# openhome/ohPipeline

Hardware: AMD Instinct MI355X
Metric: PCM Msamples/s, 256-stream 44.1->48k S24 resample+ramp+fmt (higher is better)
Workload: dtype int32

## Files before the change

include/ohgpu.h:

```cpp
#ifndef OHGPU_H
#define OHGPU_H

#include <stddef.h>
#include <stdint.h>

#ifdef __cplusplus
extern "C" {
#endif

#define OHGPU_ABI_VERSION 1

#define OHGPU_OK                0
#define OHGPU_ERR_INVALID      (-1)
#define OHGPU_ERR_DEVICE       (-2)
#define OHGPU_ERR_NO_DEVICE    (-3)
#define OHGPU_ERR_NOMEM        (-4)
#define OHGPU_ERR_BOUNDS       (-5)
#define OHGPU_ERR_UNSUPPORTED  (-6)

#define OHGPU_ENDIAN_LITTLE 1
#define OHGPU_ENDIAN_BIG    2

#define OHGPU_RAMP_MAX 16384u
#define OHGPU_UNITY_ATTENUATION 256u
// ... 800 lines not shown

int ohgpu_dsd_file_batch_check(const ohgpu_dsd_file_stream_desc* descs, size_t n, uint64_t src_arena_bytes, uint64_t dst_arena_bytes);
int ohgpu_dsd_file_batch_create(ohgpu_ctx* ctx, const ohgpu_dsd_file_stream_desc* descs, size_t n, uint64_t src_arena_bytes, uint64_t dst_arena_bytes,
                                ohgpu_batch** batch);
int ohgpu_dsd_file_batch_run(ohgpu_ctx* ctx, const ohgpu_batch* batch, const void* src_base, void* dst_base, void* stream);
int ohgpu_dsd_file_batch_results(ohgpu_ctx* ctx, const ohgpu_batch* batch, ohgpu_dsd_file_stream_result* results, size_t n);
int ohgpu_dsd_file_batch_phase_ms(ohgpu_ctx* ctx, const ohgpu_batch* batch, float ms[2]);
int ohgpu_dsd_file_process_host(ohgpu_ctx* ctx, const ohgpu_dsd_file_stream_desc* descs, size_t n, const void* src_host, uint64_t src_bytes,
                                void* dst_host, uint64_t dst_bytes, ohgpu_dsd_file_stream_result* results);
int ohgpu_dsd_file_head(const void* bytes, uint64_t n, uint32_t sample_block_words, uint32_t pad_bytes_per_chunk, ohgpu_dsd_file_stream_result* result);
int ohgpu_dsd_file_seek(uint32_t kind, uint64_t sample, uint64_t* chunk_first, uint64_t* sample_rounded);

int ohgpu_src_design(uint32_t rate_in, uint32_t rate_out, uint32_t taps_per_phase, double beta, double f_pass_hz,
                     int32_t* coef_q28, size_t coef_capacity, uint32_t* L, uint32_t* M);
int ohgpu_src_create(ohgpu_ctx* ctx, uint32_t L, uint32_t M, uint32_t taps_per_phase, const int32_t* coef_q28, ohgpu_src** src);
int ohgpu_src_destroy(ohgpu_ctx* ctx, ohgpu_src* src);
uint64_t ohgpu_src_out_frames(uint32_t L, uint32_t M, uint64_t in_frames);
int ohgpu_src_mfma_tables(uint32_t L, uint32_t M, uint32_t taps_per_phase, const int32_t* coef_q28, uint32_t max_blocks_per_row,
                          uint8_t* coef_digits, size_t coef_digits_capacity, void* steps, size_t steps_capacity,
                          size_t* coef_digits_bytes, size_t* steps_bytes, uint32_t* block_outputs);
int ohgpu_src_mfma_halfband_tables(const int32_t* coef_q28 , uint8_t* image , int64_t* bias, uint32_t* block_outputs);
int ohgpu_src_batch_create(ohgpu_ctx* ctx, const ohgpu_src* src, const ohgpu_src_msg_desc* descs, size_t n,
                           uint64_t src_arena_bytes, uint64_t dst_arena_bytes, ohgpu_batch** batch);
int ohgpu_src_batch_run(ohgpu_ctx* ctx, const ohgpu_batch* batch, const void* src_base, void* dst_base, void* stream);
int ohgpu_src_batch_run_timed(ohgpu_ctx* ctx, const ohgpu_batch* batch, const void* src_base, void* dst_base, void* stream,
                              void* start_event, void* stop_event);

int ohgpu_src_batch_block(const ohgpu_batch* batch, uint32_t* block_outputs, uint32_t* block_inputs);
int ohgpu_src_batch_advance(ohgpu_ctx* ctx, ohgpu_batch* batch, uint64_t blocks);
int ohgpu_src_batch_set_ramps(ohgpu_ctx* ctx, ohgpu_batch* batch, const uint16_t* ramp_start, const uint16_t* ramp_end, size_t n);

int ohgpu_src_process_host(ohgpu_ctx* ctx, const ohgpu_src* src, const ohgpu_src_msg_desc* descs, size_t n,
                           const void* src_host, uint64_t src_bytes, void* dst_host, uint64_t dst_bytes);

#define OHGPU_SRC_PULL_NOMINAL     (1u << 31)
#define OHGPU_SRC_PULL_MAX_STEP    (16ull << 32)

typedef struct ohgpu_src_pull_msg_desc {
    uint64_t src_offset;
    uint64_t src_frame0;
    uint64_t src_frames;
    uint64_t pos_frame;
    uint64_t step;
    uint64_t dst_offset;
    uint32_t pos_frac;
    uint32_t n_frames;
    uint16_t ramp_start;
    uint16_t ramp_end;
    uint16_t attenuation;
    uint8_t  channels;
    uint8_t  src_bits;
    uint8_t  src_endian;
    uint8_t  dst_bits;
    uint8_t  dst_endian;
    uint8_t  flags;
    uint8_t  reserved[4];
    uint64_t src_plane_stride;
} ohgpu_src_pull_msg_desc;

int ohgpu_src_pull_design(uint32_t rate_in, uint32_t rate_out, uint32_t taps_per_phase, uint32_t phases_log2, double beta,
                          double f_pass_hz, double max_pull, int32_t* coef_q28, size_t coef_capacity);
int ohgpu_src_pull_step(uint32_t rate_in, uint32_t rate_out, uint32_t multiplier, uint64_t* step);
int ohgpu_src_pull_window(uint64_t pos_frame, uint32_t pos_frac, uint64_t step, uint32_t n_frames, uint32_t taps_per_phase,
                          uint64_t* first, uint64_t* frames);
int ohgpu_src_pull_create(ohgpu_ctx* ctx, uint32_t taps_per_phase, uint32_t phases_log2, const int32_t* coef_q28, ohgpu_src** src);
int ohgpu_src_pull_destroy(ohgpu_ctx* ctx, ohgpu_src* src);
// ... 40 lines not shown
```

ohpipeline_amd/capi.py:

```python
import ctypes as C
import os

import numpy as np

_PKG = os.path.dirname(os.path.abspath(__file__))
LIB_PATH = os.path.join(_PKG, "lib", "libohgpu.so")

OK = 0
ERR_INVALID, ERR_DEVICE, ERR_NO_DEVICE, ERR_NOMEM, ERR_BOUNDS, ERR_UNSUPPORTED = -1, -2, -3, -4, -5, -6
ENDIAN_LITTLE, ENDIAN_BIG = 1, 2
RAMP_MAX = 16384
UNITY_ATTENUATION = 256
FLAG_RAMP, FLAG_SILENCE, FLAG_ZERO_LSB32, FLAG_SRC_PLANAR32 = 1, 2, 4, 8

MSG_DESC = np.dtype([
    ("src_offset", "<u8"), ("dst_offset", "<u8"), ("n_frames", "<u4"),
    ("ramp_start", "<u2"), ("ramp_end", "<u2"), ("attenuation", "<u2"),
    ("channels", "u1"), ("src_bits", "u1"), ("src_endian", "u1"),
    ("dst_bits", "u1"), ("dst_endian", "u1"), ("flags", "u1")], align=False)
SRC_MSG_DESC = np.dtype([
    ("src_offset", "<u8"), ("src_frame0", "<u8"), ("src_frames", "<u8"), ("out_frame0", "<u8"),
    ("dst_offset", "<u8"), ("n_frames", "<u4"),
    ("ramp_start", "<u2"), ("ramp_end", "<u2"), ("attenuation", "<u2"),
    ("channels", "u1"), ("src_bits", "u1"), ("src_endian", "u1"),
# ... 295 lines not shown
                                              C.c_size_t, C.POINTER(C.c_size_t)]),
    "ohgpu_flywheel_batch_create": (C.c_int, [_vp, _vp, C.c_size_t, C.c_uint64, C.c_uint64, _vpp]),
    "ohgpu_flywheel_batch_run": (C.c_int, [_vp, _vp, _vp, _vp, _vp]),
    "ohgpu_flywheel_process_host": (C.c_int, [_vp, _vp, C.c_size_t, _vp, C.c_uint64, _vp, C.c_uint64]),
    "ohgpu_ohm_frame_layout": (C.c_int, [_vp, C.c_uint32, C.POINTER(C.c_uint32), C.POINTER(C.c_uint32)]),
    "ohgpu_ohm_batch_create": (C.c_int, [_vp, _vp, C.c_size_t, _vp, C.c_size_t, _vp, C.c_size_t, C.c_uint64, C.c_uint64, _vpp]),
    "ohgpu_ohm_batch_run": (C.c_int, [_vp, _vp, _vp, _vp, _vp]),
    "ohgpu_ohm_process_host": (C.c_int, [_vp, _vp, C.c_size_t, _vp, C.c_size_t, _vp, C.c_size_t, _vp, C.c_uint64, _vp, C.c_uint64]),
    "ohgpu_src_design": (C.c_int, [C.c_uint32, C.c_uint32, C.c_uint32, C.c_double, C.c_double, _vp, C.c_size_t,
                                   C.POINTER(C.c_uint32), C.POINTER(C.c_uint32)]),
    "ohgpu_src_create": (C.c_int, [_vp, C.c_uint32, C.c_uint32, C.c_uint32, _vp, _vpp]),
    "ohgpu_src_destroy": (C.c_int, [_vp, _vp]),
    "ohgpu_src_out_frames": (C.c_uint64, [C.c_uint32, C.c_uint32, C.c_uint64]),
    "ohgpu_src_mfma_tables": (C.c_int, [C.c_uint32, C.c_uint32, C.c_uint32, _vp, C.c_uint32, _vp, C.c_size_t, _vp, C.c_size_t,
                                        C.POINTER(C.c_size_t), C.POINTER(C.c_size_t), C.POINTER(C.c_uint32)]),
    "ohgpu_src_mfma_halfband_tables": (C.c_int, [_vp, _vp, C.POINTER(C.c_int64), C.POINTER(C.c_uint32)]),
    "ohgpu_src_batch_create": (C.c_int, [_vp, _vp, _vp, C.c_size_t, C.c_uint64, C.c_uint64, _vpp]),
    "ohgpu_src_batch_run": (C.c_int, [_vp, _vp, _vp, _vp, _vp]),
    "ohgpu_src_batch_run_timed": (C.c_int, [_vp, _vp, _vp, _vp, _vp, _vp, _vp]),
    "ohgpu_src_batch_plan": (C.c_int, [_vp, _u64p, _u64p]),
    "ohgpu_src_batch_units": (C.c_int, [_vp, _u64p, _u64p]),
    "ohgpu_set_plan_threads": (C.c_int, [C.c_int]),
    "ohgpu_src_batch_block": (C.c_int, [_vp, C.POINTER(C.c_uint32), C.POINTER(C.c_uint32)]),
    "ohgpu_src_batch_advance": (C.c_int, [_vp, _vp, C.c_uint64]),
    "ohgpu_src_batch_set_ramps": (C.c_int, [_vp, _vp, _vp, _vp, C.c_size_t]),
    "ohgpu_src_plan_digest": (C.c_int, [C.c_uint32, C.c_uint32, C.c_uint32, _vp, C.c_size_t, C.c_uint64, C.c_uint64, C.c_int,
                                        _vp, C.c_int, _u64p, _u64p, _u64p, C.POINTER(C.c_int)]),
    "ohgpu_src_batch_kernel_name": (C.c_int, [_vp, _vp, C.c_char_p, C.c_size_t]),
    "ohgpu_src_batch_occupancy": (C.c_int, [_vp, _vp, C.POINTER(C.c_int), C.POINTER(C.c_int), C.POINTER(C.c_uint32)]),
    "ohgpu_measure_shader_clock": (C.c_int, [_vp, _vp, C.POINTER(C.c_double)]),
    "ohgpu_device_allocations": (C.c_int, [_vp, C.POINTER(C.c_uint64)]),
    "ohgpu_src_process_host": (C.c_int, [_vp, _vp, _vp, C.c_size_t, _vp, C.c_uint64, _vp, C.c_uint64]),
    "ohgpu_host_transfer_stats": (C.c_int, [_vp, C.POINTER(C.c_uint64), C.POINTER(C.c_uint64), C.POINTER(C.c_uint64), C.POINTER(C.c_uint64)]),
    "ohgpu_set_kernel_variant": (C.c_int, [_vp, C.c_int]),
    "ohgpu_src_pull_design": (C.c_int, [C.c_uint32, C.c_uint32, C.c_uint32, C.c_uint32, C.c_double, C.c_double, C.c_double, _vp, C.c_size_t]),
    "ohgpu_src_pull_step": (C.c_int, [C.c_uint32, C.c_uint32, C.c_uint32, _u64p]),
    "ohgpu_src_pull_window": (C.c_int, [C.c_uint64, C.c_uint32, C.c_uint64, C.c_uint32, C.c_uint32, _u64p, _u64p]),
    "ohgpu_src_pull_create": (C.c_int, [_vp, C.c_uint32, C.c_uint32, _vp, _vpp]),
    "ohgpu_src_pull_destroy": (C.c_int, [_vp, _vp]),
    "ohgpu_src_pull_batch_create": (C.c_int, [_vp, _vp, _vp, C.c_size_t, C.c_uint64, C.c_uint64, _vpp]),
    "ohgpu_src_pull_batch_run": (C.c_int, [_vp, _vp, _vp, _vp, _vp]),
    "ohgpu_src_pull_process_host": (C.c_int, [_vp, _vp, _vp, C.c_size_t, _vp, C.c_uint64, _vp, C.c_uint64]),
}
CENC_SYMBOLS = {
    "ohgpu_cenc_batch_check": (C.c_int, [_vp, C.c_size_t, C.c_size_t, C.c_size_t, C.c_uint64, C.c_uint64]),
    "ohgpu_cenc_batch_create": (C.c_int, [_vp, _vp, C.c_size_t, C.c_size_t, C.c_size_t, C.c_uint64, C.c_uint64, _vpp]),
    "ohgpu_cenc_batch_run": (C.c_int, [_vp, _vp, _vp, _vp, _vp]),
    "ohgpu_cenc_batch_results": (C.c_int, [_vp, _vp, _vp, C.c_size_t]),
    "ohgpu_cenc_batch_runs": (C.c_int, [_vp, _vp, _vp, C.c_size_t]),
    "ohgpu_cenc_batch_packets": (C.c_int, [_vp, _vp, _vp, C.c_size_t]),
    "ohgpu_cenc_batch_samples": (C.c_int, [_vp, _vp, _vp, C.c_size_t]),
    "ohgpu_cenc_batch_phase_ms": (C.c_int, [_vp, _vp, C.POINTER(C.c_float)]),
    "ohgpu_cenc_batch_paths": (C.c_int, [_vp, C.POINTER(C.c_uint32), C.POINTER(C.c_uint32), C.POINTER(C.c_uint32)]),
    "ohgpu_cenc_head": (C.c_int, [_vp, C.c_size_t, _vp]),
    "ohgpu_cenc_process_host": (C.c_int, [_vp, _vp, C.c_size_t, C.c_size_t, C.c_size_t, _vp, C.c_uint64, _vp, C.c_uint64, _vp, _vp, _vp, _vp]),
    "ohgpu_cenc_flac_process_host": (C.c_int, [_vp, _vp, _vp, C.c_size_t, C.c_size_t, C.c_size_t, _vp, C.c_uint64, C.c_uint64, _vp, C.c_uint64, _vp, _vp, _vp, _vp, _vp, _vp,
                                               C.c_size_t, C.POINTER(C.c_size_t)]),
    "ohgpu_cenc_alac_process_host": (C.c_int, [_vp, _vp, _vp, C.c_size_t, C.c_size_t, C.c_size_t, _vp, C.c_uint64, C.c_uint64, _vp, C.c_uint64, _vp, _vp, _vp, _vp, _vp, _vp]),
}
RAOP_RX_SYMBOLS = {
    "ohgpu_raop_rx_batch_check": (C.c_int, [_vp, C.c_size_t, _vp, C.c_size_t, C.c_uint64]),
    "ohgpu_raop_rx_batch_create": (C.c_int, [_vp, _vp, C.c_size_t, _vp, C.c_size_t, C.c_uint64, _vpp]),
    "ohgpu_raop_rx_batch_run": (C.c_int, [_vp, _vp, _vp, _vp]),
    "ohgpu_raop_rx_batch_results": (C.c_int, [_vp, _vp, _vp, C.c_size_t, _vp, C.c_size_t]),
    "ohgpu_raop_rx_batch_packets": (C.c_int, [_vp, _vp, _vp, C.c_size_t]),
    "ohgpu_raop_rx_batch_phase_ms": (C.c_int, [_vp, _vp, C.POINTER(C.c_float)]),
# ... 1276 lines not shown
    def src_destroy(self, src):
        check(lib().ohgpu_src_destroy(self._h, src))

    def src_batch(self, src, descs, src_arena_bytes, dst_arena_bytes):
        d = np.ascontiguousarray(descs)
        assert d.dtype == SRC_MSG_DESC
        b = C.c_void_p()
        check(lib().ohgpu_src_batch_create(self._h, src, d.ctypes.data_as(C.c_void_p), d.size, src_arena_bytes,
                                           dst_arena_bytes, C.byref(b)))
        return b

    def src_batch_block(self, batch):
        lo, mi = C.c_uint32(0), C.c_uint32(0)
        check(lib().ohgpu_src_batch_block(batch, C.byref(lo), C.byref(mi)))
        return int(lo.value), int(mi.value)

    def src_batch_advance(self, batch, blocks):
        check(lib().ohgpu_src_batch_advance(self._h, batch, blocks))

    def src_batch_set_ramps(self, batch, ramp_start, ramp_end):
        a = np.ascontiguousarray(ramp_start, dtype=np.uint16)
        e = np.ascontiguousarray(ramp_end, dtype=np.uint16)
        assert a.size == e.size
        check(lib().ohgpu_src_batch_set_ramps(self._h, batch, a.ctypes.data_as(C.c_void_p), e.ctypes.data_as(C.c_void_p), a.size))

    def src_process_host(self, src, descs, src_bytes, dst_bytes_array):
        d = np.ascontiguousarray(descs)
        assert d.dtype == SRC_MSG_DESC
        check(lib().ohgpu_src_process_host(self._h, src, d.ctypes.data_as(C.c_void_p), d.size,
                                           src_bytes.ctypes.data_as(C.c_void_p), src_bytes.nbytes,
                                           dst_bytes_array.ctypes.data_as(C.c_void_p), dst_bytes_array.nbytes))
        return dst_bytes_array

    def src_plan(self, batch):
        a, b = C.c_uint64(0), C.c_uint64(0)
        check(lib().ohgpu_src_batch_plan(batch, C.byref(a), C.byref(b)))
        return {"block_kernel_out_frames": int(a.value), "generic_pieces": int(b.value)}

    def src_units(self, batch):
        a, b = C.c_uint64(0), C.c_uint64(0)
        check(lib().ohgpu_src_batch_units(batch, C.byref(a), C.byref(b)))
        return {"units": int(a.value), "long_units": int(b.value)}

    def src_kernel_name(self, batch):
        buf = C.create_string_buffer(256)
        check(lib().ohgpu_src_batch_kernel_name(self._h, batch, buf, 256))
        return buf.value.decode()

    def src_occupancy(self, batch):
        g, want, lds = C.c_int(0), C.c_int(0), C.c_uint32(0)
        check(lib().ohgpu_src_batch_occupancy(self._h, batch, C.byref(g), C.byref(want), C.byref(lds)))
        return {"workgroups_per_cu": int(g.value), "designed_for": int(want.value), "lds_bytes": int(lds.value)}

    def device_allocations(self):
        n = C.c_uint64(0)
        check(lib().ohgpu_device_allocations(self._h, C.byref(n)))
        return int(n.value)

    def pci_bus_id(self):
        buf = C.create_string_buffer(64)
        check(lib().ohgpu_device_pci_bus_id(self._h, buf, 64))
        return buf.value.decode()

    def host_transfer_stats(self):
        v = [C.c_uint64(0) for _ in range(4)]
        check(lib().ohgpu_host_transfer_stats(self._h, *[C.byref(x) for x in v]))
# ... 41 lines not shown
```

ohpipeline_amd/csrc/api_src.hip:

```cpp
#include <cstring>
#include <string>

#include "api_common.h"
#include "src_mfma_common.h"
#include "src_plan.h"

namespace ohgpu {

struct SrcTables { std::vector<uint8_t> amat; std::vector<MfStep> steps; bool made = false; };
static bool src_describe(uint32_t L, uint32_t M, uint32_t T, const int32_t* coef_q28, ohgpu_src* s, SrcTables* tables, const char* who)
{
    int64_t max_sum_abs = 0;
    for (uint32_t p = 0; p < L; p++) {
        int64_t sabs = 0;
        for (uint32_t k = 0; k < T; k++) {
            const int32_t q = coef_q28[(size_t)p * T + k];
            sabs += q < 0 ? -(int64_t)q : (int64_t)q;
        }
        if (sabs > max_sum_abs) max_sum_abs = sabs;
        if (sabs >= ((int64_t)1 << 30)) {
            set_error(OHGPU_ERR_INVALID, "%s: phase %u has sum|c| = %lld >= 2^30 (exact fp64 accumulation bound)", who, p, (long long)sabs);
            return false;
        }
    }
// ... 123 lines not shown
            b->src_bytes_touched += r.src_bytes_touched; b->dst_bytes_written += r.dst_bytes_written;
            if (r.max_frames > b->max_frames) b->max_frames = r.max_frames;
            b->uniform = b->uniform && r.uniform;
            ordered = ordered && r.ordered;
        }
        if (n > 0) layout_of_first();
    }
    int err = OHGPU_OK;
    if (b->uniform && n > 0) err = plan_src_fast(ctx, b, descs, n, ordered, digest);
    return err;
}

enum SrcKernel { kSrcGeneric, kSrcWg, kSrcLean, kSrcBlock };
static SrcKernel src_kernel_choice(const ohgpu_ctx* ctx, const ohgpu_batch* b, bool arena_aligned = true)
{
    const int v = ctx->variant;
    if (v == 1 || !b->fast.enabled || !arena_aligned || (b->fast.wg_only && v != 0)) return kSrcGeneric;
    if (b->fast.mfma_wg && v == 0) return kSrcWg;
    if (b->fast.lean) return kSrcLean;
    if (b->fast.d_work) return kSrcBlock;
    return kSrcGeneric;
}
static const char* src_kernel_name(SrcKernel k)
{
    switch (k) {
    case kSrcWg: return "src_mfma_wg_kernel";
    case kSrcLean: return "src_lean_kernel";
    case kSrcBlock: return "src_block_kernel";
    default: return "src_kernel_v1";
    }
}
static const char* src_kernel_of(const ohgpu_ctx* ctx, const ohgpu_batch* b) { return src_kernel_name(src_kernel_choice(ctx, b)); }

}

using namespace ohgpu;

extern "C" {

int ohgpu_src_design(uint32_t rate_in, uint32_t rate_out, uint32_t taps_per_phase, double beta, double f_pass_hz,
                     int32_t* coef_q28, size_t coef_capacity, uint32_t* L, uint32_t* M)
{
    if (!L || !M) return set_error(OHGPU_ERR_INVALID, "ohgpu_src_design: null L/M");
    if (!coef_q28) return design_src(rate_in, rate_out, taps_per_phase, beta, f_pass_hz, nullptr, L, M);
    std::vector<int32_t> coef;
    const int err = design_src(rate_in, rate_out, taps_per_phase, beta, f_pass_hz, &coef, L, M);
    if (err != OHGPU_OK) return err;
    if (coef.size() > coef_capacity)
        return set_error(OHGPU_ERR_INVALID, "ohgpu_src_design: capacity %zu < L*T = %zu", coef_capacity, coef.size());
    memcpy(coef_q28, coef.data(), coef.size() * sizeof(int32_t));
    return OHGPU_OK;
}

uint64_t ohgpu_src_out_frames(uint32_t L, uint32_t M, uint64_t in_frames)
{
    if (in_frames == 0 || M == 0) return 0;
    return (in_frames * L + M - 1) / M;
}

int ohgpu_src_mfma_tables(uint32_t L, uint32_t M, uint32_t T, const int32_t* coef_q28, uint32_t max_blocks_per_row,
                          uint8_t* coef_digits, size_t coef_digits_capacity, void* steps_out, size_t steps_capacity,
                          size_t* coef_digits_bytes, size_t* steps_bytes, uint32_t* block_outputs)
{
    if (!coef_q28 || L == 0 || M == 0 || (uint64_t)L * T > (1u << 22) || max_blocks_per_row == 0 || max_blocks_per_row > 64)
        return set_error(OHGPU_ERR_INVALID, "ohgpu_src_mfma_tables: bad argument");
    std::vector<uint8_t> adig;
// ... 40 lines not shown
    ohgpu_src* s = new (std::nothrow) ohgpu_src();
    if (!s) return set_error(OHGPU_ERR_NOMEM, "ohgpu_src_create: out of host memory");
    SrcTables tables;
    if (!src_describe(L, M, T, coef_q28, s, &tables, "ohgpu_src_create")) { delete s; return OHGPU_ERR_INVALID; }
    std::vector<double> cd(n);
    for (size_t i = 0; i < n; i++) cd[i] = (double)coef_q28[i];
    hipError_t e = hipMalloc((void**)&s->d_coef, n * sizeof(double));
    if (e == hipSuccess) e = hipMalloc((void**)&s->d_coef_q28, n * sizeof(int32_t));
    if (e == hipSuccess) e = hipMemcpy(s->d_coef, cd.data(), n * sizeof(double), hipMemcpyHostToDevice);
    if (e == hipSuccess) e = hipMemcpy(s->d_coef_q28, coef_q28, n * sizeof(int32_t), hipMemcpyHostToDevice);
    if (e == hipSuccess && tables.made) {
        e = hipMalloc((void**)&s->d_mf_amat, tables.amat.size());
        if (e == hipSuccess) e = hipMalloc((void**)&s->d_mf_steps, tables.steps.size() * sizeof(MfStep));
        if (e == hipSuccess) e = hipMemcpy(s->d_mf_amat, tables.amat.data(), tables.amat.size(), hipMemcpyHostToDevice);
        if (e == hipSuccess) e = hipMemcpy(s->d_mf_steps, tables.steps.data(), tables.steps.size() * sizeof(MfStep), hipMemcpyHostToDevice);
    }
    if (e != hipSuccess) {
        if (s->d_coef) hipFree(s->d_coef);
        if (s->d_coef_q28) hipFree(s->d_coef_q28);
        if (s->d_mf_amat) hipFree(s->d_mf_amat);
        if (s->d_mf_steps) hipFree(s->d_mf_steps);
        delete s;
        return set_error(OHGPU_ERR_DEVICE, "ohgpu_src_create: %s", hipGetErrorString(e));
    }
    *out = s;
    return OHGPU_OK;
}

int ohgpu_src_destroy(ohgpu_ctx* ctx, ohgpu_src* src)
{
    CTX_GUARD("ohgpu_src_destroy");
    if (!src) return OHGPU_OK;
    if (src->pulled) return set_error(OHGPU_ERR_INVALID, "ohgpu_src_destroy: a pulled filter is destroyed with ohgpu_src_pull_destroy");
    hipFree(src->d_coef);
    hipFree(src->d_coef_q28);
    if (src->d_mf_amat) hipFree(src->d_mf_amat);
    if (src->d_mf_steps) hipFree(src->d_mf_steps);
    delete src;
    return OHGPU_OK;
}

int ohgpu_src_batch_create(ohgpu_ctx* ctx, const ohgpu_src* src, const ohgpu_src_msg_desc* descs, size_t n,
                           uint64_t src_arena_bytes, uint64_t dst_arena_bytes, ohgpu_batch** out)
{
    CTX_GUARD("ohgpu_src_batch_create");
    BatchPtr b;
    int err = batch_begin(ctx, "ohgpu_src_batch_create", kBatchSrc, src && (descs || !n), n, 0xffffffffull, src_arena_bytes, dst_arena_bytes, out, &b);
    if (err != OHGPU_OK) return err;
    if (src->pulled) return set_error(OHGPU_ERR_INVALID, "ohgpu_src_batch_create: a pulled filter (ohgpu_src_pull_create) runs through ohgpu_src_pull_batch_create");
    b->src = src;
    b->uniform = true;
    const bool keep_generic = ctx->variant == 1;
    auto convert_all = [&]() -> bool {
        b->host_descs.reset((DevSrcDesc*)host_alloc_huge((n ? n : 1) * sizeof(DevSrcDesc)));
        return b->host_descs != nullptr;
    };
    if (keep_generic && !convert_all()) return set_error(OHGPU_ERR_NOMEM, "ohgpu_src_batch_create: out of host memory");
    err = src_check_and_plan(ctx, b.get(), descs, n, b->host_descs.get(), nullptr);
    if (err != OHGPU_OK) return err;
    if (!b->uniform) {
        auto key = [](const ohgpu_src_msg_desc& d) -> uint64_t {
            return (uint64_t)d.channels | ((uint64_t)d.src_bits << 8) | ((uint64_t)d.dst_bits << 16) | ((uint64_t)d.src_endian << 24) |
                   ((uint64_t)d.dst_endian << 32) | ((uint64_t)((d.flags & OHGPU_FLAG_SRC_PLANAR32) ? 1 : 0) << 40);
        };
        std::vector<uint64_t> keys;
        std::vector<std::vector<ohgpu_src_msg_desc>> groups;
// ... 248 lines not shown
    if (f.enabled) {
        for (size_t k = 0; k < f.host_jobs.size(); k++) { f.host_jobs[k].ramp_start = ramp_start[f.job_msg[k]]; f.host_jobs[k].ramp_end = ramp_end[f.job_msg[k]]; }
        for (size_t k = 0; k < f.host_rem.size(); k++) { f.host_rem[k].ramp_start = ramp_start[f.rem_msg[k]]; f.host_rem[k].ramp_end = ramp_end[f.rem_msg[k]]; }
        if (!f.msgs_ramped.empty()) {
            for (size_t k = 0; k < f.msgs_ramped.size(); k++) {
                SegMsg& sm = f.host_msgs[f.msgs_ramped[k]];
                sm.ramp_start = ramp_start[f.msgs_ramped_msg[k]];
                sm.ramp_end = ramp_end[f.msgs_ramped_msg[k]];
            }
            OHGPU_HIP_TRY(hipMemcpyAsync(f.d_msgs, f.host_msgs.data(), f.host_msgs.size() * sizeof(SegMsg), hipMemcpyHostToDevice, s0));
        }
        if (!f.host_jobs.empty()) {
            OHGPU_HIP_TRY(hipMemcpyAsync(f.d_ramp_jobs, f.host_jobs.data(), f.host_jobs.size() * sizeof(RampJob), hipMemcpyHostToDevice, s0));
            OHGPU_HIP_TRY(hipMemsetAsync(f.d_planes, 0xff, (f.plane_entries ? f.plane_entries : 8) * sizeof(uint16_t), s0));
            OHGPU_HIP_TRY(launch_ramp_planes(ctx, f.d_ramp_jobs, (uint32_t)f.host_jobs.size(), f.d_planes, s0));
        }
        if (!f.host_rem.empty()) OHGPU_HIP_TRY(hipMemcpyAsync(f.d_rem, f.host_rem.data(), f.host_rem.size() * sizeof(DevSrcDesc), hipMemcpyHostToDevice, s0));
        if (f.planes_ready) OHGPU_HIP_TRY(hipEventRecord(f.planes_ready, s0));
        OHGPU_HIP_TRY(hipStreamSynchronize(s0));
    }
    if (b->host_descs) {
        DevSrcDesc* const dev = b->host_descs.get();
        for (size_t i = 0; i < n; i++) { dev[i].ramp_start = ramp_start[i]; dev[i].ramp_end = ramp_end[i]; }
        std::lock_guard<std::mutex> hold(b->lazy);
        if (b->d_descs) OHGPU_HIP_TRY(hipMemcpy(b->d_descs, dev, n * sizeof(DevSrcDesc), hipMemcpyHostToDevice));
    }
    return OHGPU_OK;
}

int ohgpu_src_process_host(ohgpu_ctx* ctx, const ohgpu_src* src, const ohgpu_src_msg_desc* descs, size_t n,
                           const void* src_host, uint64_t src_bytes, void* dst_host, uint64_t dst_bytes)
{
    CTX_GUARD("ohgpu_src_process_host");
    ohgpu_batch* b = nullptr;
    const int err = ohgpu_src_batch_create(ctx, src, descs, n, src_bytes, dst_bytes, &b);
    if (err != OHGPU_OK) return err;
    ctx->stage.src_calls++;
    return process_host(ctx, b, n, src_host, src_bytes, dst_host, dst_bytes, ohgpu_src_batch_run, [&](size_t i) { return frames_range(descs[i]); });
}

}
```

ohpipeline_amd/csrc/ohgpu_api.hip:

```cpp
#include <hip/hip_runtime.h>

#include <algorithm>
#include <cstdarg>
#include <cstdio>
#include <cstring>
#include <pthread.h>
#include <sched.h>

#include <atomic>
#include <condition_variable>
#include <mutex>
#include <thread>
#include <vector>

#include "api_common.h"

namespace ohgpu {

static thread_local char g_err[512] = "";
static int g_plan_threads = 0;
int plan_thread_cap() { return g_plan_threads; }

namespace {
struct PlanPool {
// ... 135 lines not shown
static int stage_reserve(ohgpu_ctx* ctx, void** p, size_t* cap, size_t bytes, bool pinned_host)
{
    if (*cap >= bytes && *p) return OHGPU_OK;
    if (*p) {
        (void)hipStreamSynchronize(ctx->stream);
        (void)(pinned_host ? hipHostFree(*p) : hipFree(*p));
        *p = nullptr; *cap = 0;
    }
    size_t want = bytes + bytes / 2;
    if (want < (64u << 10)) want = 64u << 10;
    want = (want + 4095) & ~(size_t)4095;
    const hipError_t e = pinned_host ? hipHostMalloc(p, want, hipHostMallocDefault) : hipMalloc(p, want);
    if (e != hipSuccess) {
        *p = nullptr;
        return set_error(hip_code(e), "host-buffer staging (%zu bytes): %s", want, hipGetErrorString(e));
    }
    *cap = want;
    if (!pinned_host) { std::lock_guard<std::mutex> hold(ctx->cache.m); ctx->cache.device_allocs++; }
    return OHGPU_OK;
}

int host_stage_in(ohgpu_ctx* ctx, const void* src_host, uint64_t src_bytes, uint64_t dst_bytes)
{
    HostStage& st = ctx->stage;
    st.calls++;
    int err = stage_reserve(ctx, &st.d_src, &st.src_cap, src_bytes ? src_bytes : 1, false);
    if (err == OHGPU_OK) err = stage_reserve(ctx, &st.d_dst, &st.dst_cap, dst_bytes ? dst_bytes : 1, false);
    if (err != OHGPU_OK || src_bytes == 0) return err;
    OHGPU_HIP_TRY(hipMemcpyAsync(st.d_src, src_host, src_bytes, hipMemcpyHostToDevice, ctx->stream));
    st.h2d_bytes += src_bytes;
    return OHGPU_OK;
}

int host_roundtrip(ohgpu_ctx* ctx, const void* src_host, uint64_t src_bytes, void* dst_host, uint64_t dst_bytes,
                   std::vector<std::pair<uint64_t, uint64_t>>& ranges, const std::function<int(const void*, void*)>& run)
{
    HostStage& st = ctx->stage;
    int err = host_stage_in(ctx, src_host, src_bytes, dst_bytes);
    if (err != OHGPU_OK) return err;
    hipStream_t s = ctx->stream;
    std::sort(ranges.begin(), ranges.end());
    std::vector<std::pair<uint64_t, uint64_t>> runs;
    for (const auto& r : ranges) {
        if (r.second == 0) continue;
        if (!runs.empty() && r.first <= runs.back().second) runs.back().second = std::max(runs.back().second, r.first + r.second);
        else runs.emplace_back(r.first, r.first + r.second);
    }
    err = run(st.d_src, st.d_dst);
    if (err != OHGPU_OK) { (void)hipStreamSynchronize(s); return err; }
    if (runs.empty()) { OHGPU_HIP_TRY(hipStreamSynchronize(s)); return OHGPU_OK; }
    const uint64_t lo = runs.front().first, hi = runs.back().second;
    if (runs.size() == 1) {
        OHGPU_HIP_TRY(hipMemcpyAsync((uint8_t*)dst_host + lo, (const uint8_t*)st.d_dst + lo, hi - lo, hipMemcpyDeviceToHost, s));
        st.d2h_bytes += hi - lo;
        OHGPU_HIP_TRY(hipStreamSynchronize(s));
        return OHGPU_OK;
    }
    err = stage_reserve(ctx, &st.h_bounce, &st.bounce_cap, hi - lo, true);
    if (err != OHGPU_OK) { (void)hipStreamSynchronize(s); return err; }
    OHGPU_HIP_TRY(hipMemcpyAsync(st.h_bounce, (const uint8_t*)st.d_dst + lo, hi - lo, hipMemcpyDeviceToHost, s));
    st.d2h_bytes += hi - lo;
    OHGPU_HIP_TRY(hipStreamSynchronize(s));
    for (const auto& r : runs) memcpy((uint8_t*)dst_host + r.first, (const uint8_t*)st.h_bounce + (r.first - lo), r.second - r.first);
    return OHGPU_OK;
}

int upload_batch(ohgpu_ctx* ctx, ohgpu_batch* b, const void* host_descs, size_t bytes)
{
    if (bytes == 0) return OHGPU_OK;
    hipError_t e = ctx_dev_alloc(ctx, &b->d_descs, bytes);
    if (e == hipErrorOutOfMemory) return set_error(OHGPU_ERR_NOMEM, "descriptor upload: out of device memory");
    OHGPU_HIP_TRY(e);
    e = hipMemcpy(b->d_descs, host_descs, bytes, hipMemcpyHostToDevice);
    if (e != hipSuccess) {
        ctx_dev_free(ctx, b->d_descs);
        b->d_descs = nullptr;
        return set_error(OHGPU_ERR_DEVICE, "descriptor upload: %s", hipGetErrorString(e));
    }
    return OHGPU_OK;
}
// ... 95 lines not shown
    if (!ctx) return set_error(OHGPU_ERR_NOMEM, "ohgpu_init: out of host memory");
    ctx->device = device;
    ctx->variant = 0;
    hipDeviceProp_t prop;
    hipError_t e = hipGetDeviceProperties(&prop, device);
    if (e == hipSuccess) {
        snprintf(ctx->name, sizeof(ctx->name), "%s (%s)", prop.name, prop.gcnArchName);
        ctx->num_cus = prop.multiProcessorCount;
    } else {
        snprintf(ctx->name, sizeof(ctx->name), "unknown");
        ctx->num_cus = 256;
    }
    e = hipStreamCreateWithFlags(&ctx->stream, hipStreamNonBlocking);
    if (e != hipSuccess) { delete ctx; return set_error(OHGPU_ERR_DEVICE, "hipStreamCreate: %s", hipGetErrorString(e)); }
    uint16_t table[512];
    build_ramp_table(table);
    e = hipMalloc((void**)&ctx->d_ramp_table, sizeof(table));
    if (e == hipSuccess) e = hipMemcpy(ctx->d_ramp_table, table, sizeof(table), hipMemcpyHostToDevice);
    if (e != hipSuccess) {
        hipStreamDestroy(ctx->stream);
        delete ctx;
        return set_error(OHGPU_ERR_DEVICE, "ramp table upload: %s", hipGetErrorString(e));
    }
    (void)load_ramp_plane_kernel();
    *out = ctx;
    return OHGPU_OK;
}

int ohgpu_shutdown(ohgpu_ctx* ctx)
{
    if (!ctx) return OHGPU_OK;
    hipSetDevice(ctx->device);
    hipStreamSynchronize(ctx->stream);
    hipFree(ctx->d_ramp_table);
    for (auto& list : ctx->cache.idle) for (void* p : list) (void)hipFree(p);
    if (ctx->stage.d_src) (void)hipFree(ctx->stage.d_src);
    if (ctx->stage.d_dst) (void)hipFree(ctx->stage.d_dst);
    if (ctx->stage.h_bounce) (void)hipHostFree(ctx->stage.h_bounce);
    hipStreamDestroy(ctx->stream);
    delete ctx;
    return OHGPU_OK;
}

int ohgpu_device_name(ohgpu_ctx* ctx, char* buf, size_t buf_bytes)
{
    if (!ctx || !buf || buf_bytes == 0) return set_error(OHGPU_ERR_INVALID, "ohgpu_device_name: bad argument");
    snprintf(buf, buf_bytes, "%s", ctx->name);
    return OHGPU_OK;
}

int ohgpu_device_pci_bus_id(ohgpu_ctx* ctx, char* buf, size_t buf_bytes)
{
    if (!ctx || !buf || buf_bytes < 16) return set_error(OHGPU_ERR_INVALID, "ohgpu_device_pci_bus_id: bad argument");
    OHGPU_HIP_TRY(hipDeviceGetPCIBusId(buf, (int)buf_bytes, ctx->device));
    for (char* c = buf; *c; c++) if (*c >= 'A' && *c <= 'F') *c = (char)(*c - 'A' + 'a');
    return OHGPU_OK;
}

int ohgpu_set_kernel_variant(ohgpu_ctx* ctx, int variant)
{
    if (!ctx || variant < 0 || variant > 5) return set_error(OHGPU_ERR_INVALID, "ohgpu_set_kernel_variant: bad argument");
    ctx->variant = kernel_variant_alias(variant);
    return OHGPU_OK;
}

int ohgpu_malloc(ohgpu_ctx* ctx, size_t bytes, void** dptr)
{
    CTX_GUARD("ohgpu_malloc");
    if (!dptr) return set_error(OHGPU_ERR_INVALID, "ohgpu_malloc: null out pointer");
    *dptr = nullptr;
    const hipError_t e = hipMalloc(dptr, bytes ? bytes : 1);
    if (e == hipErrorOutOfMemory) return set_error(OHGPU_ERR_NOMEM, "hipMalloc(%zu): out of device memory", bytes);
    OHGPU_HIP_TRY(e);
    return OHGPU_OK;
}

int ohgpu_free(ohgpu_ctx* ctx, void* dptr)
{
    CTX_GUARD("ohgpu_free");
    if (dptr) OHGPU_HIP_TRY(hipFree(dptr));
    return OHGPU_OK;
}

int ohgpu_malloc_host(ohgpu_ctx* ctx, size_t bytes, void** hptr)
{
    CTX_GUARD("ohgpu_malloc_host");
    if (!hptr) return set_error(OHGPU_ERR_INVALID, "ohgpu_malloc_host: null out pointer");
    OHGPU_HIP_TRY(hipHostMalloc(hptr, bytes ? bytes : 1, hipHostMallocDefault));
    return OHGPU_OK;
}

int ohgpu_free_host(ohgpu_ctx* ctx, void* hptr)
{
    CTX_GUARD("ohgpu_free_host");
// ... 255 lines not shown
```

ohpipeline_amd/csrc/ohgpu_internal.h:

```cpp
#pragma once

#include <sys/mman.h>
#include <cstdio>
#include <cstdlib>
#include <cstring>
#include <hip/hip_runtime.h>
#include <stdint.h>

#include <functional>
#include <memory>
#include <mutex>
#include <unordered_map>
#include <thread>
#include <utility>
#include <vector>

#include "../../include/ohgpu.h"
#include "alac_packet_core.h"
#include "flac_frame_core.h"
#include "ogg_page_core.h"
#include "mp4_box_core.h"
#include "mp4_frag_core.h"
#include "iff_chunk_core.h"
#include "dsd_file_core.h"
// ... 554 lines not shown
    void* d_recs = nullptr;
    void* d_floors = nullptr;
    void* d_rows = nullptr; size_t rows_bytes = 0;
    void* d_blocks = nullptr;
    void* d_cls = nullptr;
    void* d_tables = nullptr;
};
static_assert(sizeof(ohgpu_vorbis_stream_desc) == 64 && sizeof(ohgpu_vorbis_packet_result) == sizeof(vorbiscore::Rec) && sizeof(ohgpu_vorbis_stream_result) == 24 &&
              sizeof(ohgpu_vorbis_info) == 32 && offsetof(ohgpu_vorbis_packet_result, position) == offsetof(vorbiscore::Rec, position) &&
              offsetof(ohgpu_vorbis_packet_result, reserved) == offsetof(vorbiscore::Rec, prev_block) && vorbiscore::kMaxCoupling == OHGPU_VORBIS_MAX_COUPLING_STEPS &&
              vorbiscore::kMaxImageBytes == OHGPU_VORBIS_MAX_IMAGE_BYTES && vorbiscore::kMaxClassBytes == OHGPU_VORBIS_MAX_CLASS_BYTES, "Vorbis layouts");

enum BatchKind { kBatchPcm = 1, kBatchSrc = 2, kBatchFmt = 3, kBatchFlywheel = 4, kBatchOhm = 5, kBatchSrcPull = 6, kBatchDsd = 7, kBatchFlac = 8, kBatchDsdPcm = 9, kBatchAlac = 10, kBatchRaop = 11, kBatchOhmRx = 12, kBatchOgg = 13, kBatchMp4 = 14, kBatchIff = 15, kBatchDsdFile = 16, kBatchMp4f = 17, kBatchCenc = 18, kBatchRaopRx = 19, kBatchTs = 20, kBatchAdts = 21, kBatchVorbis = 22 };

}

namespace ohgpu {
struct DevCache {
    static constexpr int kClasses = 15;
    std::mutex m;
    std::vector<void*> idle[kClasses];
    std::unordered_map<void*, int> cls;
    uint64_t device_allocs = 0;
};
}

namespace ohgpu {
struct HostStage {
    void*  d_src = nullptr;    size_t src_cap = 0;
    void*  d_dst = nullptr;    size_t dst_cap = 0;
    void*  h_bounce = nullptr; size_t bounce_cap = 0;
    uint64_t h2d_bytes = 0, d2h_bytes = 0, calls = 0, src_calls = 0;
};
}

struct ohgpu_ctx {
    ohgpu::DevCache cache;
    ohgpu::HostStage stage;
    int          device;
    hipStream_t  stream;
    uint16_t*    d_ramp_table;
    int          variant;
    int          num_cus;
    char         name[128];
};

struct ohgpu_src {
    uint32_t L, M, T;
    int64_t  max_sum_abs;
    bool     halfband;
    double*  d_coef;
    int32_t* d_coef_q28;
    uint8_t* d_mf_amat = nullptr;
    ohgpu::MfStep* d_mf_steps = nullptr;
    uint32_t mf_L_blk = 0;
    bool     mf_halfband = false;
    bool     pulled = false;
    uint32_t phases_log2 = 0;
    int32_t* d_pull_table = nullptr;
};

struct ohgpu_dsd_pcm {
    uint32_t D, T, N;
    int32_t* d_coef = nullptr;
    int32_t* d_tables = nullptr;
};

namespace ohgpu {
struct HostFree { void operator()(void* p) const { free(p); } };
inline void* host_alloc_huge(size_t bytes)
{
// ... 108 lines not shown
int  raop_rx_plan(ohgpu_ctx* ctx, ohgpu_batch* b, const raoprx::Stream* streams, const raoprx::Datagram* datagrams);
int  raop_rx_run(ohgpu_ctx* ctx, const ohgpu_batch* b, const uint8_t* src, hipStream_t s);
int  ts_plan(ohgpu_ctx* ctx, ohgpu_batch* b, const tspkt::Stream* streams);
int  ts_run(ohgpu_ctx* ctx, const ohgpu_batch* b, const uint8_t* src, uint8_t* dst, hipStream_t s);
uint32_t ts_wave_blocks(uint64_t tiles, uint32_t cus);
int  adts_plan(ohgpu_ctx* ctx, ohgpu_batch* b, const adts::Stream* streams);
int  adts_run(ohgpu_ctx* ctx, const ohgpu_batch* b, const uint8_t* src, hipStream_t s);
int  vorbis_plan(ohgpu_ctx* ctx, ohgpu_batch* b, const void* images, uint64_t images_bytes);
int  vorbis_run(ohgpu_ctx* ctx, const ohgpu_batch* b, const uint8_t* src, uint8_t* dst, hipStream_t s);
int  ogg_plan(ohgpu_ctx* ctx, ohgpu_batch* b, const oggpage::Stream* streams);
int  ogg_run(ohgpu_ctx* ctx, const ohgpu_batch* b, const uint8_t* src, uint8_t* dst, hipStream_t s);
uint32_t ogg_wave_blocks(uint64_t items, uint32_t cus);
int  mp4_plan(ohgpu_ctx* ctx, ohgpu_batch* b, const mp4box::Stream* streams);
int  mp4_run(ohgpu_ctx* ctx, const ohgpu_batch* b, const uint8_t* src, hipStream_t s);
int  mp4f_plan(ohgpu_ctx* ctx, Mp4fState& g, const mp4frag::Stream* streams, const char* who);
int  mp4f_run(ohgpu_ctx* ctx, const ohgpu_batch* b, const uint8_t* src, uint8_t* dst, hipStream_t s);
int  mp4f_tables(const Mp4fState& g, const uint8_t* src, hipStream_t s);
uint32_t mp4f_wave_blocks(uint64_t slots, uint32_t cus);
int  cenc_plan(ohgpu_ctx* ctx, ohgpu_batch* b, const cenc::Stream* streams);
int  cenc_run(ohgpu_ctx* ctx, const ohgpu_batch* b, const uint8_t* src, uint8_t* dst, hipStream_t s);
void cenc_free(ohgpu_ctx* ctx, ohgpu_batch* b);
int  iff_plan(ohgpu_ctx* ctx, ohgpu_batch* b, const iffchunk::Stream* streams);
int  iff_run(ohgpu_ctx* ctx, const ohgpu_batch* b, const uint8_t* src, uint8_t* dst, hipStream_t s);
int  dsd_file_plan(ohgpu_ctx* ctx, ohgpu_batch* b, const dsdfile::Stream* streams);
int  dsd_file_run(ohgpu_ctx* ctx, const ohgpu_batch* b, const uint8_t* src, uint8_t* dst, hipStream_t s);
OhmSelRec wide_record(uint64_t src_off, uint64_t dst_off, uint32_t n_frames, uint32_t channels, uint32_t sb, bool little, uint64_t src_arena_bytes);
hipError_t launch_ohm_wide(const ohgpu_ctx* ctx, const void* d_recs, uint32_t n_recs, const uint8_t* src, uint8_t* dst, const uint8_t* prefix, hipStream_t s);
int plan_flywheel(ohgpu_ctx* ctx, ohgpu_batch* b, const ohgpu_flywheel_desc* descs, size_t n);
void free_flywheel(ohgpu_ctx* ctx, ohgpu_batch* b);
hipError_t ctx_dev_alloc(ohgpu_ctx* ctx, void** p, size_t bytes);
void ctx_dev_free(ohgpu_ctx* ctx, void* p);
int host_roundtrip(ohgpu_ctx* ctx, const void* src_host, uint64_t src_bytes, void* dst_host, uint64_t dst_bytes,
                   std::vector<std::pair<uint64_t, uint64_t>>& ranges, const std::function<int(const void* d_src, void* d_dst)>& run);
hipError_t launch_flywheel(const ohgpu_ctx* ctx, const ohgpu_batch* b, const uint8_t* src, uint8_t* dst, hipStream_t s);
hipError_t launch_src_v1(const ohgpu_ctx* ctx, const void* d_descs, size_t n, const ohgpu_src* src_filter,
                         const uint8_t* src, uint8_t* dst, hipStream_t s);
hipError_t launch_src_block(const ohgpu_ctx* ctx, const ohgpu_batch* b, const uint8_t* src, uint8_t* dst, hipStream_t s);
hipError_t launch_src_lean(const ohgpu_ctx* ctx, const ohgpu_batch* b, const uint8_t* src, uint8_t* dst, hipStream_t s);
struct WgOccupancy { bool query = true; int groups_per_cu = 0, designed_for = 0; uint32_t lds_bytes = 0; hipEvent_t start = nullptr, stop = nullptr; };
hipError_t launch_src_mfma_wg(const ohgpu_ctx* ctx, const ohgpu_batch* b, const uint8_t* src, uint8_t* dst, hipStream_t s, WgOccupancy* query = nullptr);
bool src_mfma_wg_supported(uint32_t L_blk, uint32_t M_blk, uint32_t ch, uint32_t sb, uint32_t db, bool planar, bool halfband);
bool src_mfma_wg_unit_inside(int64_t src_row0, uint32_t row_src_bytes, uint64_t src_arena_bytes, uint32_t ch, uint32_t sb, uint32_t unit_rows, bool planar, uint64_t plane_stride, bool halfband);
bool build_mfma_halfband(const int32_t* coef_q28, uint32_t L_blk, std::vector<MfStep>* steps, std::vector<uint8_t>* amat);
bool build_mfma_tables(uint32_t L, uint32_t M, uint32_t T, const int32_t* coef_q28, uint32_t L_blk, uint32_t kb_cap,
                       std::vector<uint8_t>* adig, std::vector<MfStep>* steps);
void build_mfma_images(const std::vector<uint8_t>& adig, const std::vector<MfStep>& steps, uint32_t L, std::vector<uint8_t>* amat);
bool src_mfma_supported(uint32_t T, uint32_t ch, uint32_t sb, uint32_t db);
uint32_t src_block_outputs(uint32_t L, uint32_t fb_dst);
hipError_t launch_ramp_planes(const ohgpu_ctx* ctx, const void* d_jobs, uint32_t n_jobs, void* d_planes, hipStream_t s);
hipError_t load_ramp_plane_kernel();
bool src_lean_geometry(uint32_t L, uint32_t T, bool halfband, uint32_t ch, uint32_t sb, uint32_t db, uint32_t out_per_drain,
                       uint32_t* rows, uint32_t* in_blocks, uint32_t* stage_frames, uint32_t* ring_bytes, uint32_t* coef_lds_bytes,
                       uint32_t* wave_lds_bytes, uint32_t* max_waves);
bool src_block_supported(uint32_t T, uint32_t ch, uint32_t sb, uint32_t src_le, uint32_t db, uint32_t dst_le);
bool src_block_built(uint32_t T, uint32_t ch, uint32_t sb, uint32_t src_le, uint32_t db, uint32_t dst_le);
bool src_lean_only_supported(uint32_t T, uint32_t ch, uint32_t sb, uint32_t src_le, uint32_t db, uint32_t dst_le);
bool src_lean_halfband_supported(uint32_t T, uint32_t ch, uint32_t sb, uint32_t src_le, uint32_t db, uint32_t dst_le);
bool src_block_geometry(uint32_t L, uint32_t T, uint32_t ch, uint32_t sb, uint32_t db, uint32_t out_per_drain,
                        uint32_t* rows, uint32_t* ring_bytes, uint32_t* coef_lds_bytes, uint32_t* wave_lds_bytes, uint32_t* max_waves);

constexpr uint32_t kPullTile = 256;
struct PullTile {
    uint32_t msg;
    uint32_t j0;
    uint32_t count;
    uint32_t win_frames;
// ... 34 lines not shown
```

Before: 397,600.

## Cache live SRC batches across host process calls and advance instead of rebuilding

Adds a small LRU cache of SRC batch plans inside the context, keyed on the filter and the descriptor shape. When a later host call matches, it advances the cached batch by whole blocks and re-applies ramps instead of creating a new batch, and it reuses the precomputed transfer runs. This removes per-call batch planning and allocation on the host. In exchange the descriptors must be compared on every call, and a new cache state has to be invalidated on filter destroy and on variant changes.

```diff
diff --git a/include/ohgpu.h b/include/ohgpu.h
--- a/include/ohgpu.h
+++ b/include/ohgpu.h
@@ -856,6 +856,8 @@
 
 int ohgpu_src_process_host(ohgpu_ctx* ctx, const ohgpu_src* src, const ohgpu_src_msg_desc* descs, size_t n,
                            const void* src_host, uint64_t src_bytes, void* dst_host, uint64_t dst_bytes);
+int ohgpu_src_live_cache_set(ohgpu_ctx* ctx, size_t entries);
+int ohgpu_src_live_cache_stats(ohgpu_ctx* ctx, uint64_t* hits, uint64_t* misses, size_t* entries);
 
 #define OHGPU_SRC_PULL_NOMINAL     (1u << 31)
 #define OHGPU_SRC_PULL_MAX_STEP    (16ull << 32)
diff --git a/ohpipeline_amd/capi.py b/ohpipeline_amd/capi.py
--- a/ohpipeline_amd/capi.py
+++ b/ohpipeline_amd/capi.py
@@ -351,6 +351,8 @@
     "ohgpu_device_allocations": (C.c_int, [_vp, C.POINTER(C.c_uint64)]),
     "ohgpu_src_process_host": (C.c_int, [_vp, _vp, _vp, C.c_size_t, _vp, C.c_uint64, _vp, C.c_uint64]),
     "ohgpu_host_transfer_stats": (C.c_int, [_vp, C.POINTER(C.c_uint64), C.POINTER(C.c_uint64), C.POINTER(C.c_uint64), C.POINTER(C.c_uint64)]),
+    "ohgpu_src_live_cache_set": (C.c_int, [_vp, C.c_size_t]),
+    "ohgpu_src_live_cache_stats": (C.c_int, [_vp, C.POINTER(C.c_uint64), C.POINTER(C.c_uint64), C.POINTER(C.c_size_t)]),
     "ohgpu_set_kernel_variant": (C.c_int, [_vp, C.c_int]),
     "ohgpu_src_pull_design": (C.c_int, [C.c_uint32, C.c_uint32, C.c_uint32, C.c_uint32, C.c_double, C.c_double, C.c_double, _vp, C.c_size_t]),
     "ohgpu_src_pull_step": (C.c_int, [C.c_uint32, C.c_uint32, C.c_uint32, _u64p]),
@@ -1693,6 +1695,14 @@
                                            dst_bytes_array.ctypes.data_as(C.c_void_p), dst_bytes_array.nbytes))
         return dst_bytes_array
 
+    def src_live_cache_set(self, entries):
+        check(lib().ohgpu_src_live_cache_set(self._h, entries))
+
+    def src_live_cache_stats(self):
+        h, m, e = C.c_uint64(0), C.c_uint64(0), C.c_size_t(0)
+        check(lib().ohgpu_src_live_cache_stats(self._h, C.byref(h), C.byref(m), C.byref(e)))
+        return {"hits": int(h.value), "misses": int(m.value), "entries": int(e.value)}
+
     def src_plan(self, batch):
         a, b = C.c_uint64(0), C.c_uint64(0)
         check(lib().ohgpu_src_batch_plan(batch, C.byref(a), C.byref(b)))
diff --git a/ohpipeline_amd/csrc/api_src.hip b/ohpipeline_amd/csrc/api_src.hip
--- a/ohpipeline_amd/csrc/api_src.hip
+++ b/ohpipeline_amd/csrc/api_src.hip
@@ -179,6 +179,75 @@
 }
 static const char* src_kernel_of(const ohgpu_ctx* ctx, const ohgpu_batch* b) { return src_kernel_name(src_kernel_choice(ctx, b)); }
 
+static void live_entry_destroy(ohgpu_ctx* ctx, LiveEntry& e)
+{
+    if (e.batch) (void)ohgpu_batch_destroy(ctx, e.batch);
+    e.batch = nullptr;
+}
+void live_cache_clear(ohgpu_ctx* ctx)
+{
+    for (LiveEntry& e : ctx->live.entries) live_entry_destroy(ctx, e);
+    ctx->live.entries.clear();
+}
+void live_cache_drop_filter(ohgpu_ctx* ctx, const ohgpu_src* src)
+{
+    std::vector<LiveEntry>& v = ctx->live.entries;
+    for (size_t i = v.size(); i-- > 0;)
+        if (v[i].src == src) { live_entry_destroy(ctx, v[i]); v.erase(v.begin() + (ptrdiff_t)i); }
+}
+static void live_cache_trim(ohgpu_ctx* ctx, size_t keep)
+{
+    std::vector<LiveEntry>& v = ctx->live.entries;
+    while (v.size() > keep) {
+        size_t old = 0;
+        for (size_t i = 1; i < v.size(); i++) if (v[i].used < v[old].used) old = i;
+        live_entry_destroy(ctx, v[old]);
+        v.erase(v.begin() + (ptrdiff_t)old);
+    }
+}
+enum LiveMatch { kLiveMiss, kLiveHit, kLiveMoved, kLiveRefused };
+static LiveMatch live_match(const LiveEntry& e, const ohgpu_src* src, const ohgpu_src_msg_desc* descs, size_t n, uint64_t src_bytes, uint64_t dst_bytes,
+                            uint64_t* blocks, bool* reramp, int* err)
+{
+    if (e.src != src || e.descs.size() != n || e.src_bytes != src_bytes || e.dst_bytes != dst_bytes) return kLiveMiss;
+    uint64_t k = 0;
+    bool moved = false;
+    *reramp = false;
+    for (size_t i = 0; i < n; i++) {
+        const ohgpu_src_msg_desc& d = descs[i];
+        const ohgpu_src_msg_desc& o = e.descs[i];
+        if (d.channels != o.channels || d.src_bits != o.src_bits || d.dst_bits != o.dst_bits || d.src_endian != o.src_endian || d.dst_endian != o.dst_endian ||
+            d.flags != o.flags || d.attenuation != o.attenuation || d.n_frames != o.n_frames || d.src_frames != o.src_frames || d.src_offset != o.src_offset ||
+            d.dst_offset != o.dst_offset || d.src_plane_stride != o.src_plane_stride) return kLiveMiss;
+        if (d.out_frame0 < o.out_frame0 || d.src_frame0 < o.src_frame0) return kLiveMiss;
+        const uint64_t d_out = d.out_frame0 - o.out_frame0, d_in = d.src_frame0 - o.src_frame0;
+        uint64_t ki = 0;
+        if (e.block_outputs == 0) moved = moved || d_out != 0 || d_in != 0;
+        else if (d_out != 0 || d_in != 0) {
+            if (d_out % e.block_outputs != 0) return kLiveMiss;
+            ki = d_out / e.block_outputs;
+            if (d_in != ki * e.block_inputs) return kLiveMiss;
+        }
+        if (i == 0) k = ki;
+        else if (ki != k) return kLiveMiss;
+        if (d.ramp_start > OHGPU_RAMP_MAX || d.ramp_end > OHGPU_RAMP_MAX) { *err = set_error(OHGPU_ERR_INVALID, "src desc %zu: ramp beyond Ramp::kMax", i); return kLiveRefused; }
+        if (d.out_frame0 > (1ull << 48) || d.src_frame0 > (1ull << 48)) { *err = set_error(OHGPU_ERR_INVALID, "src desc %zu: frame index out of range", i); return kLiveRefused; }
+        if ((d.flags & OHGPU_FLAG_RAMP) && (d.ramp_start != o.ramp_start || d.ramp_end != o.ramp_end)) *reramp = true;
+    }
+    *blocks = k;
+    return moved ? kLiveMoved : kLiveHit;
+}
+static void live_block(const ohgpu_batch* b, uint32_t* block_outputs, uint32_t* block_inputs)
+{
+    *block_outputs = *block_inputs = 0;
+    const ohgpu_batch* p = b->parts.empty() ? b : b->parts[0];
+    if (!p->fast.enabled) return;
+    for (const ohgpu_batch* q : b->parts)
+        if (!q->fast.enabled || q->fast.params.L_blk != p->fast.params.L_blk) return;
+    *block_outputs = p->fast.params.L_blk;
+    *block_inputs = p->fast.params.M_blk;
+}
+
 }
 
 using namespace ohgpu;
@@ -285,6 +354,7 @@
     CTX_GUARD("ohgpu_src_destroy");
     if (!src) return OHGPU_OK;
     if (src->pulled) return set_error(OHGPU_ERR_INVALID, "ohgpu_src_destroy: a pulled filter is destroyed with ohgpu_src_pull_destroy");
+    live_cache_drop_filter(ctx, src);
     hipFree(src->d_coef);
     hipFree(src->d_coef_q28);
     if (src->d_mf_amat) hipFree(src->d_mf_amat);
@@ -599,11 +669,91 @@
                            const void* src_host, uint64_t src_bytes, void* dst_host, uint64_t dst_bytes)
 {
     CTX_GUARD("ohgpu_src_process_host");
+    LiveCache& live = ctx->live;
+    auto roundtrip = [&](const ohgpu_batch* batch, const std::vector<std::pair<uint64_t, uint64_t>>& runs) {
+        ctx->stage.src_calls++;
+        return host_roundtrip_runs(ctx, src_host, src_bytes, dst_host, dst_bytes, runs,
+                                   [&](const void* d_src, void* d_dst) { return ohgpu_src_batch_run(ctx, batch, d_src, d_dst, nullptr); });
+    };
+    size_t stale = live.entries.size();
+    if (src && descs && n > 0) {
+        for (size_t at = 0; at < live.entries.size(); at++) {
+            LiveEntry& e = live.entries[at];
+            uint64_t blocks = 0;
+            bool reramp = false;
+            int err = OHGPU_OK;
+            const LiveMatch m = live_match(e, src, descs, n, src_bytes, dst_bytes, &blocks, &reramp, &err);
+            if (m == kLiveRefused) return err;
+            if (m == kLiveMiss) continue;
+            stale = at;
+            if (!e.batch) { if (m == kLiveHit) live.barren = 0; break; }
+            if (m == kLiveMoved) break;
+            if (blocks > 0 && ohgpu_src_batch_advance(ctx, e.batch, blocks) != OHGPU_OK) break;
+            if (reramp) {
+                std::vector<uint16_t> ramps(2 * n);
+                for (size_t i = 0; i < n; i++) { ramps[i] = descs[i].ramp_start; ramps[n + i] = descs[i].ramp_end; }
+                err = ohgpu_src_batch_set_ramps(ctx, e.batch, ramps.data(), ramps.data() + n, n);
+                if (err == OHGPU_ERR_UNSUPPORTED) break;
+                if (err != OHGPU_OK) return err;
+            }
+            memcpy(e.descs.data(), descs, n * sizeof(ohgpu_src_msg_desc));
+            e.used = ++live.clock;
+            live.hits++;
+            live.barren = 0;
+            return roundtrip(e.batch, e.runs);
+        }
+    }
     ohgpu_batch* b = nullptr;
     const int err = ohgpu_src_batch_create(ctx, src, descs, n, src_bytes, dst_bytes, &b);
     if (err != OHGPU_OK) return err;
-    ctx->stage.src_calls++;
-    return process_host(ctx, b, n, src_host, src_bytes, dst_host, dst_bytes, ohgpu_src_batch_run, [&](size_t i) { return frames_range(descs[i]); });
-}
-
-}
+    if (live.cap == 0 || n == 0) {
+        ctx->stage.src_calls++;
+        return process_host(ctx, b, n, src_host, src_bytes, dst_host, dst_bytes, ohgpu_src_batch_run, [&](size_t i) { return frames_range(descs[i]); });
+    }
+    live.misses++;
+    const bool keep = live.barren < 2 * live.cap;
+    if (keep) live.barren++;
+    else for (LiveEntry& e : live.entries) live_entry_destroy(ctx, e);
+    if (stale < live.entries.size()) live_entry_destroy(ctx, live.entries[stale]);
+    else {
+        live_cache_trim(ctx, live.cap - 1);
+        live.entries.emplace_back();
+        stale = live.entries.size() - 1;
+    }
+    LiveEntry& e = live.entries[stale];
+    e.src = src;
+    e.src_bytes = src_bytes; e.dst_bytes = dst_bytes;
+    e.descs.assign(descs, descs + n);
+    live_block(b, &e.block_outputs, &e.block_inputs);
+    std::vector<std::pair<uint64_t, uint64_t>> out(n);
+    for (size_t i = 0; i < n; i++) out[i] = frames_range(descs[i]);
+    host_merge_runs(out, &e.runs);
+    e.used = ++live.clock;
+    if (keep) e.batch = b;
+    const BatchPtr once(keep ? nullptr : b, BatchDeleter{ctx});
+    return roundtrip(b, e.runs);
+}
+
+int ohgpu_src_live_cache_set(ohgpu_ctx* ctx, size_t entries)
+{
+    CTX_GUARD("ohgpu_src_live_cache_set");
+    if (entries > 64) return set_error(OHGPU_ERR_INVALID, "ohgpu_src_live_cache_set: %zu entries (at most 64)", entries);
+    ctx->live.cap = entries;
+    ctx->live.barren = 0;
+    live_cache_trim(ctx, entries);
+    return OHGPU_OK;
+}
+
+int ohgpu_src_live_cache_stats(ohgpu_ctx* ctx, uint64_t* hits, uint64_t* misses, size_t* entries)
+{
+    if (!ctx) return set_error(OHGPU_ERR_INVALID, "ohgpu_src_live_cache_stats: null context");
+    if (hits) *hits = ctx->live.hits;
+    if (misses) *misses = ctx->live.misses;
+    if (entries) {
+        *entries = 0;
+        for (const LiveEntry& e : ctx->live.entries) *entries += e.batch ? 1 : 0;
+    }
+    return OHGPU_OK;
+}
+
+}
diff --git a/ohpipeline_amd/csrc/ohgpu_api.hip b/ohpipeline_amd/csrc/ohgpu_api.hip
--- a/ohpipeline_amd/csrc/ohgpu_api.hip
+++ b/ohpipeline_amd/csrc/ohgpu_api.hip
@@ -191,20 +191,32 @@
     return OHGPU_OK;
 }
 
+void host_merge_runs(std::vector<std::pair<uint64_t, uint64_t>>& ranges, std::vector<std::pair<uint64_t, uint64_t>>* runs)
+{
+    std::sort(ranges.begin(), ranges.end());
+    runs->clear();
+    for (const auto& r : ranges) {
+        if (r.second == 0) continue;
+        if (!runs->empty() && r.first <= runs->back().second) runs->back().second = std::max(runs->back().second, r.first + r.second);
+        else runs->emplace_back(r.first, r.first + r.second);
+    }
+}
+
 int host_roundtrip(ohgpu_ctx* ctx, const void* src_host, uint64_t src_bytes, void* dst_host, uint64_t dst_bytes,
                    std::vector<std::pair<uint64_t, uint64_t>>& ranges, const std::function<int(const void*, void*)>& run)
+{
+    std::vector<std::pair<uint64_t, uint64_t>> runs;
+    host_merge_runs(ranges, &runs);
+    return host_roundtrip_runs(ctx, src_host, src_bytes, dst_host, dst_bytes, runs, run);
+}
+
+int host_roundtrip_runs(ohgpu_ctx* ctx, const void* src_host, uint64_t src_bytes, void* dst_host, uint64_t dst_bytes,
+                        const std::vector<std::pair<uint64_t, uint64_t>>& runs, const std::function<int(const void*, void*)>& run)
 {
     HostStage& st = ctx->stage;
     int err = host_stage_in(ctx, src_host, src_bytes, dst_bytes);
     if (err != OHGPU_OK) return err;
     hipStream_t s = ctx->stream;
-    std::sort(ranges.begin(), ranges.end());
-    std::vector<std::pair<uint64_t, uint64_t>> runs;
-    for (const auto& r : ranges) {
-        if (r.second == 0) continue;
-        if (!runs.empty() && r.first <= runs.back().second) runs.back().second = std::max(runs.back().second, r.first + r.second);
-        else runs.emplace_back(r.first, r.first + r.second);
-    }
     err = run(st.d_src, st.d_dst);
     if (err != OHGPU_OK) { (void)hipStreamSynchronize(s); return err; }
     if (runs.empty()) { OHGPU_HIP_TRY(hipStreamSynchronize(s)); return OHGPU_OK; }
@@ -366,6 +378,7 @@
     if (!ctx) return OHGPU_OK;
     hipSetDevice(ctx->device);
     hipStreamSynchronize(ctx->stream);
+    live_cache_clear(ctx);
     hipFree(ctx->d_ramp_table);
     for (auto& list : ctx->cache.idle) for (void* p : list) (void)hipFree(p);
     if (ctx->stage.d_src) (void)hipFree(ctx->stage.d_src);
@@ -394,6 +407,10 @@
 int ohgpu_set_kernel_variant(ohgpu_ctx* ctx, int variant)
 {
     if (!ctx || variant < 0 || variant > 5) return set_error(OHGPU_ERR_INVALID, "ohgpu_set_kernel_variant: bad argument");
+    if (kernel_variant_alias(variant) != ctx->variant) {
+        OHGPU_HIP_TRY(hipSetDevice(ctx->device));
+        live_cache_clear(ctx);
+    }
     ctx->variant = kernel_variant_alias(variant);
     return OHGPU_OK;
 }
diff --git a/ohpipeline_amd/csrc/ohgpu_internal.h b/ohpipeline_amd/csrc/ohgpu_internal.h
--- a/ohpipeline_amd/csrc/ohgpu_internal.h
+++ b/ohpipeline_amd/csrc/ohgpu_internal.h
@@ -610,11 +610,27 @@
     void*  h_bounce = nullptr; size_t bounce_cap = 0;
     uint64_t h2d_bytes = 0, d2h_bytes = 0, calls = 0, src_calls = 0;
 };
+struct LiveEntry {
+    ohgpu_batch* batch = nullptr;
+    const ohgpu_src* src = nullptr;
+    uint64_t src_bytes = 0, dst_bytes = 0;
+    std::vector<ohgpu_src_msg_desc> descs;
+    std::vector<std::pair<uint64_t, uint64_t>> runs;
+    uint32_t block_outputs = 0, block_inputs = 0;
+    uint64_t used = 0;
+};
+struct LiveCache {
+    std::vector<LiveEntry> entries;
+    size_t   cap = 4;
+    uint64_t hits = 0, misses = 0, clock = 0;
+    size_t   barren = 0;
+};
 }
 
 struct ohgpu_ctx {
     ohgpu::DevCache cache;
     ohgpu::HostStage stage;
+    ohgpu::LiveCache live;
     int          device;
     hipStream_t  stream;
     uint16_t*    d_ramp_table;
@@ -789,6 +805,11 @@
 void ctx_dev_free(ohgpu_ctx* ctx, void* p);
 int host_roundtrip(ohgpu_ctx* ctx, const void* src_host, uint64_t src_bytes, void* dst_host, uint64_t dst_bytes,
                    std::vector<std::pair<uint64_t, uint64_t>>& ranges, const std::function<int(const void* d_src, void* d_dst)>& run);
+void host_merge_runs(std::vector<std::pair<uint64_t, uint64_t>>& ranges, std::vector<std::pair<uint64_t, uint64_t>>* runs);
+int host_roundtrip_runs(ohgpu_ctx* ctx, const void* src_host, uint64_t src_bytes, void* dst_host, uint64_t dst_bytes,
+                        const std::vector<std::pair<uint64_t, uint64_t>>& runs, const std::function<int(const void* d_src, void* d_dst)>& run);
+void live_cache_clear(ohgpu_ctx* ctx);
+void live_cache_drop_filter(ohgpu_ctx* ctx, const ohgpu_src* src);
 hipError_t launch_flywheel(const ohgpu_ctx* ctx, const ohgpu_batch* b, const uint8_t* src, uint8_t* dst, hipStream_t s);
 hipError_t launch_src_v1(const ohgpu_ctx* ctx, const void* d_descs, size_t n, const ohgpu_src* src_filter,
                          const uint8_t* src, uint8_t* dst, hipStream_t s);
```

New measurement: 400,600, median of 3. About the same (+0.8%).
